# hku-mars/BALM

Measured on AMD Instinct MI355X. Metric: BA iterations/sec (W poses x F plane features), higher is better.
Workload: dtype f64

## Files before the change

balm_amd/csrc/balm_capi.hip:

```cpp
#include <algorithm>
#include <array>
#include <atomic>
#include <chrono>
#include <cmath>
#include <cstdio>
#include <cstdlib>
#include <cstring>

#include "balm_internal.h"

using namespace balm;

#define HIP_TRY(expr)                                                                              \
  do {                                                                                             \
    hipError_t e_ = (expr);                                                                        \
    if (e_ != hipSuccess) {                                                                        \
      ctx->err = std::string(#expr) + ": " + hipGetErrorString(e_);                                \
      return BALM_ERR_HIP;                                                                         \
    }                                                                                              \
  } while (0)

namespace {

#ifdef BALM_COLD_TRACE
// ... 40 lines not shown

static void adopt_warm_ring(balm_ctx *ctx) {
  if (ctx->ring.buf[0] || ctx->device < 0 || ctx->device >= 64) return;
  DeviceWarm &w = g_warm[ctx->device];
  std::lock_guard<std::mutex> lk(w.mu);
  if (!w.started) return;
  if (w.th.joinable()) w.th.join();
  if (w.ring_ready.load(std::memory_order_acquire)) {
    const int key = ctx->ring.pool_key;
    ctx->ring = w.ring; ctx->ring.pool_key = key;
    w.ring = PinnedRing(); w.ring_ready.store(false);
  }
}

struct Span {
  balm_ctx *c; int slot; hipEvent_t a = nullptr, b = nullptr;
  Span(balm_ctx *ctx, int s) : c(ctx), slot(s) {
    if (!c->timer.on) return;
    a = take(); b = take();
    hipEventRecord(a, c->stream);
  }
  ~Span() {
    if (!c->timer.on) return;
    hipEventRecord(b, c->stream);
    c->timer.pending.push_back({a, b, slot});
  }
  hipEvent_t take() {
    if (!c->timer.pool.empty()) { hipEvent_t e = c->timer.pool.back(); c->timer.pool.pop_back(); return e; }
    hipEvent_t e; hipEventCreate(&e); return e;
  }
};

void collect_timing(balm_ctx *c) {
  for (auto &sp : c->timer.pending) {
    float ms = 0;
    if (hipEventElapsedTime(&ms, sp.a, sp.b) == hipSuccess) { c->timer.ms[sp.slot] += ms; c->timer.cnt[sp.slot]++; }
    c->timer.pool.push_back(sp.a); c->timer.pool.push_back(sp.b);
  }
  c->timer.pending.clear();
}

template <class T>
int dalloc(balm_ctx *ctx, T **p, size_t count) {
  if (*p) { hipFree(*p); *p = nullptr; }
  if (count == 0) count = 1;
  HIP_TRY(hipMalloc((void **)p, count * sizeof(T)));
  return BALM_OK;
}

template <class T>
int keep(balm_ctx *ctx, T **p, size_t *cap, size_t count) {
  if (*p && *cap >= count) return BALM_OK;
  for (int k = 0; k < balm_ctx::LM_GRAPHS; k++)
    if (ctx->lm_graph[k]) { hipGraphExecDestroy(ctx->lm_graph[k]); ctx->lm_graph[k] = nullptr; ctx->lm_graph_form[k] = -1; }
// ... 31 lines not shown
  return reinterpret_cast<T *>(ctx->d_stage + off);
}

int sync_stream(balm_ctx *ctx) {
  HIP_TRY(hipStreamSynchronize(ctx->stream));
  HIP_TRY(hipGetLastError());
  collect_timing(ctx);
  return BALM_OK;
}

long red_dacc_off(const balm_ctx *c) { return (long)c->ntiles * TILE_ELEMS; }
long red_r_off(const balm_ctx *c) { return red_dacc_off(c) + (long)DACC_MAX * c->W; }

bool has_transport(const balm_ctx *ctx) { return ctx->comm || multi_is_loopback(ctx) || ctx->allreduce; }

int hook_allreduce(balm_ctx *ctx, double *buf, long n) {
  if (ctx->comm) { Span sp(ctx, BALM_T_COMM); return comm_allreduce(ctx, buf, n); }
  if (multi_is_loopback(ctx)) { Span sp(ctx, BALM_T_COMM); return loopback_allreduce(ctx, buf, n); }
  if (!ctx->allreduce) return BALM_OK;
  int rc = sync_stream(ctx);
  if (rc) return rc;
  if (ctx->allreduce((void *)buf, n, ctx->allreduce_user) != 0) {
    ctx->err = "all-reduce hook failed";
    return BALM_ERR_STATE;
  }
  return BALM_OK;
}

int set_damping(balm_ctx *ctx, double u) {
  ctx->u_value = u;
  ctx->u_on_device = false;
  return BALM_OK;
}
int push_damping(balm_ctx *ctx) {
  double *slot = ctx->h_scal + 16 + (ctx->u_ring++ & 63);
  *slot = ctx->u_value;
  HIP_TRY(hipMemcpyAsync(ctx->d_scal + SCAL_U, slot, sizeof(double), hipMemcpyHostToDevice, ctx->stream));
  ctx->u_on_device = true;
  return BALM_OK;
}

static void collect_timing_if_idle(balm_ctx *ctx) {
  if (!ctx->timer.on || ctx->timer.pending.empty()) return;
  if (hipStreamSynchronize(ctx->stream) == hipSuccess) collect_timing(ctx);
}

int wait_scalars(balm_ctx *ctx) {
  volatile double *stamp = ctx->h_scal + SCAL_STAMP;
  const double want = (double)ctx->mail_seq;
  const auto t0 = std::chrono::steady_clock::now();
  for (int spin = 0;; spin++) {
    if (*stamp == want) { std::atomic_thread_fence(std::memory_order_acquire); collect_timing_if_idle(ctx); return BALM_OK; }
    if ((spin & 255) == 255 && std::chrono::steady_clock::now() - t0 > std::chrono::microseconds(300)) break;
  }
  int rc = sync_stream(ctx);
  if (rc) return rc;
  if (*stamp != want) { ctx->err = "balm_damping_iter: the iteration's scalars did not arrive"; return BALM_ERR_HIP; }
  return BALM_OK;
}

void drop_lm_graphs(balm_ctx *ctx) {
  for (int k = 0; k < balm_ctx::LM_GRAPHS; k++) {
    if (ctx->lm_graph[k]) hipGraphExecDestroy(ctx->lm_graph[k]);
    ctx->lm_graph[k] = nullptr; ctx->lm_graph_form[k] = -1;
  }
}

int residual_device(balm_ctx *ctx, const double *d_poses, int f0, int f1, int slot, bool defer_sum = false, bool send_mail = false) {
  if (f1 <= f0) {
    HIP_TRY(hipMemsetAsync(ctx->d_scal + slot, 0, sizeof(double), ctx->stream));
    ctx->nr_tmp = 0;
  } else {
    Span sp(ctx, BALM_T_MOMENTS);
    launch_world_moments(ctx->stream, ctx->d_cl, d_poses, ctx->W, f0, f1, ctx->d_C);
    const EigenMail mail{ctx->d_scal, ctx->d_hscal, send_mail ? (double)++ctx->mail_seq : 0.0, slot};
    ctx->nr_tmp = launch_feature_eigen(ctx->stream, ctx->d_C, ctx->has_fix ? ctx->d_fix : nullptr, ctx->d_coe, f0, f1, ctx->d_feat_tmp,
                                       ctx->d_rpart_tmp, send_mail ? &mail : nullptr);
    if (!defer_sum) launch_sum_scalar(ctx->stream, ctx->d_rpart_tmp, ctx->nr_tmp, ctx->d_scal + slot);
  }
  HIP_TRY(hipGetLastError());
  if (defer_sum) return BALM_OK;
  return hook_allreduce(ctx, ctx->d_scal + slot, 1);
}

bool fuse_trial(const balm_ctx *ctx) {
  const char *e = getenv("BALM_FUSE_TRIAL");
  return ctx->W <= 256 && ctx->F > 0 && e && e[0] == '1';
}

static bool syrk_int8_mode(const balm_ctx *ctx) {
  if (ctx->flags & BALM_FLAG_SYRK_INT8) return true;
  const char *m = getenv("BALM_SYRK");
  return m && !strcmp(m, "int8");
}
static bool syrk_int8_for(const balm_ctx *ctx, long K) {
  if (!syrk_int8_mode(ctx)) return false;
  if (const char *m = getenv("BALM_SYRK_INT8_MIN_COLS")) return K >= atol(m);
  return K >= 12288L && ctx->W >= 96;
}

int prepare_evaluate(balm_ctx *ctx, int form, int nf) {
  if (nf <= 0) return BALM_OK;
  const SyrkPlan plan = plan_syrk(ctx->ntiles, 3L * nf);
  int rc;
  size_t gcols = (size_t)plan.Kpad + 64, parts = (size_t)plan.SG * ctx->ntiles;
  if (ctx->sparse && nf == ctx->F) {
    gcols = (size_t)ctx->sp_nchunks * ctx->sp_nsteps * 4 + 64;
    parts = (size_t)ctx->sp_nitems;
  }
  {
    const double *before = ctx->d_Gt;
    if ((rc = ensure(ctx, &ctx->d_Gt, &ctx->cap_Gt, gcols * ctx->npad))) return rc;
// ... 6 lines not shown
    if (!ctx->d_rowmax2) ctx->rowmax_trial_valid = false;
    if ((rc = ensure(ctx, &ctx->d_rowmax, &ctx->cap_rowmax, (size_t)ctx->npad + 128))) return rc;
    if ((rc = ensure(ctx, &ctx->d_rowmax2, &ctx->cap_rowmax2, (size_t)ctx->npad + 128))) return rc;
    if ((rc = ensure(ctx, &ctx->d_rowmax_part, &ctx->cap_rowmax_part, (size_t)factors_grid(ctx->W, nf, form) * 6 * ctx->W))) return rc;
    HIP_TRY(prepare_device_syrk_i8());
  }
  if ((rc = ensure(ctx, &ctx->d_dpart, &ctx->cap_dpart, (size_t)factors_grid(ctx->W, nf, form) * DACC_MAX * ctx->W))) return rc;
  if (nf == ctx->F && fuse_trial(ctx)) {
    if (ctx->cap_Gt2 < gcols * ctx->npad || ctx->cap_dpart2 < (size_t)factors_grid(ctx->W, nf, form) * DACC_MAX * ctx->W) ctx->gt_trial_valid = false;
    if ((rc = ensure(ctx, &ctx->d_Gt2, &ctx->cap_Gt2, gcols * ctx->npad))) return rc;
    if ((rc = ensure(ctx, &ctx->d_dpart2, &ctx->cap_dpart2, (size_t)factors_grid(ctx->W, nf, form) * DACC_MAX * ctx->W))) return rc;
  }
  return BALM_OK;
}

int evaluate_device(balm_ctx *ctx, int form, const double *d_poses, int f0, int f1, int slot) {
  const int W = ctx->W, nf = f1 - f0;
  const int dacc = form == 0 ? DACC_LEFT : DACC_RIGHT;
  int rc;
  if (nf <= 0) {
    HIP_TRY(hipMemsetAsync(ctx->d_red, 0, ctx->red_len * sizeof(double), ctx->stream));
    if ((rc = hook_allreduce(ctx, ctx->d_red, (long)ctx->red_len))) return rc;
    Span sp(ctx, BALM_T_ASSEMBLE);
    launch_assemble(ctx->stream, form, ctx->d_red, red_dacc_off(ctx), ctx->d_sub, ctx->ntiles, W, ctx->d_H, ctx->d_g,
                    ctx->d_red + red_r_off(ctx), ctx->d_scal + slot);
    return BALM_OK;
  }
  SyrkPlan plan = plan_syrk(ctx->ntiles, 3L * nf);
  if ((rc = prepare_evaluate(ctx, form, nf))) return rc;
  const int nblk = factors_grid(W, nf, form);
  hipStream_t s = ctx->stream;
  if (!(ctx->feat_cur_valid && f0 == 0 && f1 == ctx->F)) {
    Span sp(ctx, BALM_T_MOMENTS);
    launch_world_moments(s, ctx->d_cl, d_poses, W, f0, f1, ctx->d_C);
    ctx->nr_cur = launch_feature_eigen(s, ctx->d_C, ctx->has_fix ? ctx->d_fix : nullptr, ctx->d_coe, f0, f1, ctx->d_feat, ctx->d_rpart);
    ctx->feat_cur_valid = (f0 == 0 && f1 == ctx->F);
  }
  const int nr = ctx->nr_cur;
  const bool sparse = ctx->sparse && f0 == 0 && f1 == ctx->F;
  const size_t kpad = sparse ? (size_t)ctx->sp_nchunks * ctx->sp_nsteps * 4 : (size_t)plan.Kpad;
  if (!(ctx->gt_cur_valid && ctx->feat_cur_valid && f0 == 0 && f1 == ctx->F)) {
    Span sp(ctx, BALM_T_FACTORS);
    const size_t k0 = (size_t)3 * nf, k1 = kpad + 64;
    if (ctx->gt_dirty_cols == ~(size_t)0) {
      HIP_TRY(hipMemsetAsync(ctx->d_Gt, 0, ctx->cap_Gt * sizeof(double), s));
      ctx->gt_dirty_cols = 0;
    } else if (ctx->gt_dirty_cols > k0) {
      HIP_TRY(hipMemsetAsync(ctx->d_Gt + k0 * ctx->npad, 0, (std::max(ctx->gt_dirty_cols, k1) - k0) * ctx->npad * sizeof(double), s));
    }
    ctx->gt_dirty_cols = k0;
    ctx->rowmax_cur_valid = launch_factors(s, form, ctx->d_cl, d_poses, ctx->d_feat, W, ctx->npad, f0, f1, ctx->d_Gt, ctx->d_dpart, nblk,
                                           sparse ? ctx->d_slot : nullptr, (!sparse && syrk_int8_for(ctx, 3L * nf)) ? ctx->d_rowmax : nullptr, ctx->d_rowmax_part);
    ctx->gt_cur_valid = false;
  }
  HIP_TRY(hipGetLastError());
  const bool int8 = !sparse && syrk_int8_for(ctx, 3L * nf);
  {
    Span sp(ctx, BALM_T_SYRK);
    if (sparse) launch_syrk_sparse(s, ctx->d_Gt, ctx->npad, ctx->d_jobs, ctx->d_items, ctx->d_chunk_ids, ctx->sp_nsteps, ctx->sp_nitems, ctx->d_part);
    else if (int8) {
      if (launch_syrk_i8(s, ctx->d_Gt, ctx->npad, ctx->n, 3L * nf, ctx->d_sub, ctx->ntiles, ctx->d_i8, ctx->d_part,
                         ctx->rowmax_cur_valid ? ctx->d_rowmax : nullptr)) { ctx->err = "INT8 SYRK: unsupported size"; return BALM_ERR_ARG; }
      plan.SG = 1;
    }
    else launch_syrk(s, ctx->d_Gt, ctx->npad, ctx->ntiles, ctx->d_jobs, plan, ctx->d_part);
  }
  {
    Span sp(ctx, BALM_T_ASSEMBLE);
    launch_reduce(s, ctx->d_part, plan.SG, (long)ctx->ntiles * TILE_ELEMS, ctx->d_dpart, nblk, dacc * W,
                  ctx->d_rpart, nr, ctx->d_red, red_dacc_off(ctx), red_r_off(ctx), sparse ? ctx->d_csr : nullptr);
  }
  if ((rc = hook_allreduce(ctx, ctx->d_red, (long)ctx->red_len))) return rc;
  {
    Span sp(ctx, BALM_T_ASSEMBLE);
    launch_assemble(s, form, ctx->d_red, red_dacc_off(ctx), ctx->d_sub, ctx->ntiles, W, ctx->d_H, ctx->d_g, ctx->d_red + red_r_off(ctx),
                    ctx->d_scal + slot);
  }
  return BALM_OK;
}

int trial_device(balm_ctx *ctx, int form, const double *d_poses, int slot) {
  const int W = ctx->W, F = ctx->F;
  hipStream_t s = ctx->stream;
  const SyrkPlan plan = plan_syrk(ctx->ntiles, 3L * F);
  const bool sparse = ctx->sparse;
  const size_t kpad = sparse ? (size_t)ctx->sp_nchunks * ctx->sp_nsteps * 4 : (size_t)plan.Kpad;
  const int nblk = factors_grid(W, F, form);
  {
    Span sp(ctx, BALM_T_FACTORS);
    const size_t k0 = (size_t)3 * F, k1 = kpad + 64;
    HIP_TRY(hipMemsetAsync(ctx->d_Gt2 + k0 * ctx->npad, 0, (k1 - k0) * ctx->npad * sizeof(double), s));
    if (ctx->npad > ctx->n)
      HIP_TRY(hipMemset2DAsync(ctx->d_Gt2 + ctx->n, (size_t)ctx->npad * sizeof(double), 0,
                               (size_t)(ctx->npad - ctx->n) * sizeof(double), k0, s));
    ctx->nr_tmp = launch_moments_factors(s, form, ctx->d_cl, d_poses, ctx->has_fix ? ctx->d_fix : nullptr, ctx->d_coe, W, ctx->npad, F,
                                         ctx->d_Gt2, ctx->d_dpart2, nblk, sparse ? ctx->d_slot : nullptr, ctx->d_feat_tmp, ctx->d_rpart_tmp,
                                         (!sparse && syrk_int8_for(ctx, 3L * F) && ctx->d_rowmax2) ? ctx->d_rowmax2 : nullptr, ctx->d_rowmax_part);
    ctx->rowmax_trial_valid = !sparse && syrk_int8_for(ctx, 3L * F) && ctx->d_rowmax2;
  }
  HIP_TRY(hipGetLastError());
  {
    Span sp(ctx, BALM_T_MOMENTS);
    launch_sum_scalar(s, ctx->d_rpart_tmp, ctx->nr_tmp, ctx->d_scal + slot);
  }
  ctx->gt_trial_valid = true;
  return hook_allreduce(ctx, ctx->d_scal + slot, 1);
}

int read_scalars(balm_ctx *ctx) {
  HIP_TRY(hipMemcpyAsync(ctx->h_scal, ctx->d_scal, 16 * sizeof(double), hipMemcpyDeviceToHost, ctx->stream));
  return sync_stream(ctx);
}

std::vector<unsigned char> obs_of(const double *clusters, int F, int W) {
  std::vector<unsigned char> obs((size_t)F * W);
  parallel_ranges(obs.size(), (size_t)1 << 16, [&](size_t lo, size_t hi) {
    for (size_t t = lo; t < hi; t++) obs[t] = clusters[t * 10 + 9] != 0 ? 1 : 0;
  });
  return obs;
}

// ... 53 lines not shown
  if (hipGetDeviceCount(&ndev) != hipSuccess || ndev < 1 || device < 0 || device >= ndev) return nullptr;
  if (hipSetDevice(device) != hipSuccess) return nullptr;
  cold_mark("balm_create: hipGetDeviceCount + hipSetDevice");
  warm_start(device);
  if (prepare_device_accum() != hipSuccess || prepare_device_cov() != hipSuccess) return nullptr;
  cold_mark("balm_create: prepare_device (function attributes -> code objects)");
  balm_ctx *ctx = new balm_ctx();
  ctx->W = win_size;
  ctx->n = 6 * win_size;
  ctx->npad = (ctx->n + TILE - 1) / TILE * TILE;
  ctx->T = ctx->npad / TILE;
  ctx->nA = (ctx->n + NB - 1) / NB * NB;
  ctx->device = device;
  ctx->flags = flags;
  ctx->timer.on = (flags & BALM_FLAG_TIMING) != 0;
  auto fail = [&]() -> balm_ctx * { one_destroy(ctx); return nullptr; };
  std::vector<int> jobs, sub;
  {
    const int T = ctx->T, ngroups = T / 5;
    std::vector<std::array<int, 3>> mixed[4];
    std::vector<std::array<int, 2>> pairs;
    for (int r = 0; r < TM; r++) for (int c = r; c < TM; c++) pairs.push_back({r, c});
    for (int k = 0; k < 15; k++) mixed[1].push_back({0, pairs[k][0], pairs[k][1]});
    for (int k = 0; k < 10; k++) mixed[1].push_back({1, pairs[k][0], pairs[k][1]});
    for (int k = 10; k < 15; k++) mixed[2].push_back({1, pairs[k][0], pairs[k][1]});
    for (int k = 0; k < 15; k++) mixed[2].push_back({2, pairs[k][0], pairs[k][1]});
    for (int k = 0; k < 5; k++) mixed[2].push_back({3, pairs[k][0], pairs[k][1]});
    for (int k = 5; k < 15; k++) mixed[3].push_back({3, pairs[k][0], pairs[k][1]});
    for (int k = 0; k < 15; k++) mixed[3].push_back({4, pairs[k][0], pairs[k][1]});
    auto regular = [&](int I, int J) {
// ... 54 lines not shown
  if (!ctx) return;
  if (ctx->counted_live) { context_gone(ctx->device); ctx->counted_live = false; }
  comm_destroy(ctx);
  drop_lm_graphs(ctx);
  hipSetDevice(ctx->device);
  if (ctx->stream) hipStreamSynchronize(ctx->stream);
  if (ctx->window) { window_close(ctx->window); ctx->window = nullptr; }
  void *ptrs[] = {ctx->d_cl, ctx->d_fix, ctx->d_coe, ctx->d_poses, ctx->d_poses_tmp, ctx->d_C, ctx->d_feat,
                  ctx->d_Gt, ctx->d_Gt2, ctx->d_dpart2, ctx->d_part, ctx->d_dpart, ctx->d_rpart, ctx->d_feat_tmp, ctx->d_rpart_tmp, ctx->d_red, ctx->d_jobs, ctx->d_sub, ctx->d_H,
                  ctx->d_g, ctx->d_A, ctx->d_Wp, ctx->d_dvec, ctx->d_z, ctx->d_x, ctx->d_perm, ctx->d_dx, ctx->d_scal, ctx->d_arena, ctx->d_pre, ctx->d_flags, ctx->d_minv, ctx->d_macro_tab, ctx->d_trace, ctx->d_slot, ctx->d_items, ctx->d_csr, ctx->d_chunk_ids, ctx->d_stage, ctx->d_i8, ctx->d_rowmax, ctx->d_rowmax2, ctx->d_rowmax_part};
  for (void *p : ptrs) if (p) hipFree(p);
  if (ctx->h_scal) hipHostFree(ctx->h_scal);
  ctx->ring.release();
  if (ctx->amail.host) hipHostFree((void *)ctx->amail.host);
  if (ctx->amail.scan_state) hipFree(ctx->amail.scan_state);
  for (auto &sp : ctx->timer.pending) { hipEventDestroy(sp.a); hipEventDestroy(sp.b); }
  for (auto e : ctx->timer.pool) hipEventDestroy(e);
  if (ctx->stream) hipStreamDestroy(ctx->stream);
  delete ctx;
}

static int build_sparse_plan(balm_ctx *ctx, int F, const unsigned char *obs) {
  ctx->sparse = false;
  const char *mode = getenv("BALM_SYRK");
  if (mode && !strcmp(mode, "dense")) return BALM_OK;
  if (syrk_int8_for(ctx, 3L * F)) return BALM_OK;
  const int W = ctx->W, T = ctx->T, ntiles = ctx->ntiles;
  if (T > 128 || T <= 2 || F < 64) return BALM_OK;
  struct Key { uint64_t hi, lo; int a; };
  std::vector<Key> keys((size_t)F);
  parallel_ranges((size_t)F, (size_t)(65536 / W + 1), [&](size_t a0, size_t a1) {
    for (size_t a = a0; a < a1; a++) {
      uint64_t hi = 0, lo = 0;
      const unsigned char *oa = obs + a * W;
      for (int i = 0; i < W; i++)
        if (oa[i])
          for (int b = (6 * i) / TILE; b <= (6 * i + 5) / TILE; b++) {
            if (b < 64) hi |= 1ull << (63 - b); else lo |= 1ull << (127 - b);
// ... 72 lines not shown
  drop_lm_graphs(ctx);
  ctx->has_fix = fix != nullptr;
  if (fix) {
    if ((rc = keep(ctx, &ctx->d_fix, &ctx->cap_fix, (size_t)F * 10))) return rc;
    HIP_TRY(hipMemcpyAsync(ctx->d_fix, fix, (size_t)F * 10 * sizeof(double), kind, ctx->stream));
  }
  if ((rc = keep(ctx, &ctx->d_coe, &ctx->cap_coe, (size_t)F))) return rc;
  HIP_TRY(hipMemcpyAsync(ctx->d_coe, coeffs, (size_t)F * sizeof(double), kind, ctx->stream));
  if ((rc = keep(ctx, &ctx->d_C, &ctx->cap_C, (size_t)F * 10))) return rc;
  if ((rc = keep(ctx, &ctx->d_feat, &ctx->cap_feat, (size_t)F * FEAT_STRIDE))) return rc;
  if ((rc = keep(ctx, &ctx->d_feat_tmp, &ctx->cap_feat_tmp, (size_t)F * FEAT_STRIDE))) return rc;
  if ((rc = keep(ctx, &ctx->d_rpart, &ctx->cap_rpart, (size_t)(F + 255) / 256 + 1024 + 1))) return rc;
  if ((rc = keep(ctx, &ctx->d_rpart_tmp, &ctx->cap_rpart_tmp, (size_t)(F + 255) / 256 + 1024 + 1))) return rc;
  ctx->feat_cur_valid = false; ctx->gt_cur_valid = false;
  ctx->F = F;
  return BALM_OK;
}

static int assoc_clusters_host(balm_ctx *ctx);

using FillClusters = std::function<void(int, int, double *, unsigned char *)>;

static int one_set_features_fn(balm_ctx *ctx, int F, const FillClusters &fill, const double *fix, const double *coeffs, bool shard_books = false) {
  if (!ctx) return BALM_ERR_ARG;
  if (ctx->multi && F == 0) { ctx->F = 0; ctx->feat_cur_valid = false; ctx->gt_cur_valid = false; ctx->planes_per_pose.clear(); ctx->work_S = ctx->work_B = 0; return BALM_OK; }
  if (F < 1 || !fill || !coeffs) { ctx->err = "balm_set_features: bad argument"; return BALM_ERR_ARG; }
  HIP_TRY(hipSetDevice(ctx->device));
  const int W = ctx->W;
  const size_t count = (size_t)F * W * 10;
  int rc;
// ... 585 lines not shown
  if (!std::isfinite(ctx->h_scal[2]) && !ctx->persistent_off && solve_timed_out(ctx)) {
    ctx->persistent_off = true;
    {
      Span sp(ctx, BALM_T_SOLVE);
      launch_solve(ctx, true);
    }
    HIP_TRY(hipMemcpyAsync(dxi, ctx->d_dx, (size_t)n * sizeof(double), hipMemcpyDeviceToHost, ctx->stream));
    if ((rc = read_scalars(ctx))) return rc;
  }
  if (q1) *q1 = ctx->h_scal[2];
  return BALM_OK;
}

static int lm_enqueue(balm_ctx *ctx, int form, bool evaluated, bool mail) {
  int rc;
  if (evaluated && (rc = evaluate_device(ctx, form, ctx->d_poses, 0, ctx->F, 0))) return rc;
  {
    Span sp(ctx, BALM_T_SOLVE);
    launch_solve(ctx, evaluated, form, ctx->d_poses, ctx->d_poses_tmp);
  }
  ctx->gt_trial_valid = false;
  bool sum_in_mail = false;
  if (fuse_trial(ctx) && ctx->d_Gt2 && ctx->d_dpart2) {
    if ((rc = trial_device(ctx, form, ctx->d_poses_tmp, 1))) return rc;
  } else {
    sum_in_mail = mail && !has_transport(ctx) && ctx->F > 0;
    const bool eigen_mails = sum_in_mail && ctx->F <= 256;
    if ((rc = residual_device(ctx, ctx->d_poses_tmp, 0, ctx->F, 1, sum_in_mail, eigen_mails))) return rc;
    if (eigen_mails) return BALM_OK;
  }
  if (mail) launch_scalars_mail(ctx->stream, ctx->d_scal, ctx->d_hscal, (double)++ctx->mail_seq, sum_in_mail ? ctx->d_rpart_tmp : nullptr,
                                ctx->nr_tmp, 1);
  else HIP_TRY(hipMemcpyAsync(ctx->h_scal, ctx->d_scal, 16 * sizeof(double), hipMemcpyDeviceToHost, ctx->stream));
  return BALM_OK;
}

static int lm_iteration(balm_ctx *ctx, int form, bool evaluated, int it) {
  const char *genv = getenv("BALM_GRAPH");
  const bool disabled = !(genv && (!strcmp(genv, "1") || !strcmp(genv, "debug")));
  const bool graphable = !disabled && ctx->graphs_ok && it >= 1 && !ctx->timer.on && !has_transport(ctx) && !ctx->multi &&
                         ctx->feat_cur_valid && ctx->F > 0 && !solve_is_persistent(ctx);
  if (graphable) {
    const bool fused = fuse_trial(ctx) && ctx->d_Gt2 && ctx->d_dpart2;
    const int slot = (ctx->gt_parity ? 16 : 0) | (fused ? 8 : 0) | (ctx->gt_cur_valid ? 4 : 0) | (evaluated ? 2 : 0) | ctx->parity;
    if (ctx->lm_graph[slot] && ctx->lm_graph_form[slot] != form) {
      hipGraphExecDestroy(ctx->lm_graph[slot]); ctx->lm_graph[slot] = nullptr;
    }
    if (!ctx->lm_graph[slot]) {
      hipGraph_t g = nullptr;
      ctx->u_on_device = true;
      bool ok = hipStreamBeginCapture(ctx->stream, hipStreamCaptureModeThreadLocal) == hipSuccess;
      if (ok) {
        const int rc = lm_enqueue(ctx, form, evaluated, false);
        const hipError_t e = hipStreamEndCapture(ctx->stream, &g);
        ok = rc == BALM_OK && e == hipSuccess && g != nullptr;
      }
      if (ok) ok = hipGraphInstantiate(&ctx->lm_graph[slot], g, nullptr, nullptr, 0) == hipSuccess;
      if (g) hipGraphDestroy(g);
      if (genv && !strcmp(genv, "debug")) fprintf(stderr, "balm_hip: LM graph slot %d capture %s\n", slot, ok ? "ok" : "FAILED");
      if (!ok) {
        hipGetLastError();
        ctx->lm_graph[slot] = nullptr;
        ctx->graphs_ok = false;
      } else {
        ctx->lm_graph_form[slot] = form;
      }
    }
    if (ctx->lm_graph[slot]) {
      int rcu = push_damping(ctx);
      if (rcu) return rcu;
      HIP_TRY(hipGraphLaunch(ctx->lm_graph[slot], ctx->stream));
      return sync_stream(ctx);
    }
    ctx->u_on_device = false;
  }
  int rc = lm_enqueue(ctx, form, evaluated, true);
  if (rc) return rc;
  return wait_scalars(ctx);
}

static int one_damping_iter(balm_ctx *ctx, const balm_lm_opts *o, double *poses, balm_iter_log *log, int *n_iters) {
  if (!ctx) return BALM_ERR_ARG;
  if (!ctx->multi && ctx->F < 1) { ctx->err = "balm_damping_iter: no features installed"; return BALM_ERR_STATE; }
  if (!o || !poses || (o->form != 0 && o->form != 1) || o->max_iter < 1) {
    ctx->err = "balm_damping_iter: bad argument"; return BALM_ERR_ARG;
  }
  if (n_iters) *n_iters = 0;
  HIP_TRY(hipSetDevice(ctx->device));
  const int W = ctx->W, F = ctx->F;
  hipStream_t s = ctx->stream;
  cold_mark("damping_iter: enter");
  int rc = prepare_evaluate(ctx, o->form, F);
// ... 453 lines not shown
  });
}

int balm_get_solve_trace(balm_ctx *ctx, long long *ticks, long capacity, int *dims3) {
  if (!ctx || !dims3) return BALM_ERR_ARG;
  const int P = ctx->nA / NB, RB = 2 * P + 1;
  dims3[0] = RB; dims3[1] = P; dims3[2] = 6;
  if (!ctx->d_trace) { ctx->err = "balm_get_solve_trace: create the context with BALM_SOLVE_TRACE=1 in the environment"; return BALM_ERR_STATE; }
  if (!ticks || capacity < (long)RB * P * 6 + 6L * P) { ctx->err = "balm_get_solve_trace: buffer too small"; return BALM_ERR_ARG; }
  HIP_TRY(hipSetDevice(ctx->device));
  HIP_TRY(hipStreamSynchronize(ctx->stream));
  HIP_TRY(hipMemcpy(ticks, ctx->d_trace, ((size_t)RB * P * 6 + 6 * (size_t)P) * sizeof(long long), hipMemcpyDeviceToHost));
  return BALM_OK;
}

int balm_get_timing(balm_ctx *ctx, double *ms, long *count) {
  if (!ctx) return BALM_ERR_ARG;
  for (int k = 0; k < BALM_T_COUNT; k++) {
    if (ms) ms[k] = ctx->timer.ms[k];
    if (count) count[k] = ctx->timer.cnt[k];
  }
  return BALM_OK;
}

int balm_get_shard_timing(balm_ctx *ctx, int shard, double *ms, long *count) {
  if (!ctx) return BALM_ERR_ARG;
  balm_ctx *q = ctx;
  if (ctx->multi) {
    if (shard < 0 || shard >= ctx->multi->n) { ctx->err = "balm_get_shard_timing: no such shard"; return BALM_ERR_ARG; }
    q = ctx->multi->sub[(size_t)shard];
  } else if (shard != 0) { ctx->err = "balm_get_shard_timing: no such shard"; return BALM_ERR_ARG; }
  return balm_get_timing(q, ms, count);
}

int balm_chain_macro_plan(int panels, int helpers, int *table, long capacity) {
  if (!table || panels < 3 || helpers < 1 || capacity < (long)helpers * 64) return BALM_ERR_ARG;
  std::vector<int> tab;
  if (!balm::chain_macro_plan(panels, helpers, tab)) return BALM_ERR_ARG;
  memcpy(table, tab.data(), tab.size() * sizeof(int));
  return BALM_OK;
}

int balm_reset_timing(balm_ctx *ctx) {
  if (!ctx) return BALM_ERR_ARG;
  for (int k = 0; k < BALM_T_COUNT; k++) { ctx->timer.ms[k] = 0; ctx->timer.cnt[k] = 0; }
  if (balm_multi *m = leader_of(ctx))
    for (size_t q = 1; q < m->sub.size(); q++)
      for (int k = 0; k < BALM_T_COUNT; k++) { m->sub[q]->timer.ms[k] = 0; m->sub[q]->timer.cnt[k] = 0; }
  return BALM_OK;
}

int balm_work_model(balm_ctx *ctx, double *out4) {
  if (!ctx || !out4) return BALM_ERR_ARG;
  const double W = ctx->W, F = ctx->multi ? ctx->multi->F : ctx->F;
  out4[0] = ctx->work_S;
  out4[1] = ctx->work_B;
  if (ctx->multi && ctx->multi->books_per_shard) {
    out4[0] = out4[1] = 0;
    for (const balm_ctx *q : ctx->multi->sub) { out4[0] += q->work_S; out4[1] += q->work_B; }
  }
  (void)W;
  out4[2] = 216.0 * out4[1];
  SyrkPlan p = plan_syrk(ctx->ntiles, 3L * (long)F);
// ... 17 lines not shown
```

balm_amd/csrc/balm_internal.h:

```cpp
#pragma once
#include <hip/hip_runtime.h>
#include <atomic>
#include <condition_variable>
#include <cstddef>
#include <cstdint>
#include <functional>
#include <mutex>
#include <string>
#include <thread>
#include <vector>

#include "../../include/balm_hip.h"
#include "host_stage.h"

namespace balm {

constexpr int TILE = 80;
constexpr int TM = 5;
constexpr int TILE_ELEMS = TILE * TILE;
constexpr int FEAT_STRIDE = 24;
constexpr int DACC_LEFT = 27;
constexpr int DACC_RIGHT = 30;
constexpr int DACC_MAX = 30;
constexpr int NB = 48;
constexpr int MAX_W_LDS = 480;
constexpr int MAX_W = 1024;
constexpr int MAX_SHARDS = 16;

enum { FT_NN = 0, FT_VBAR = 1, FT_LAM = 4, FT_U0 = 7, FT_U1 = 10, FT_U2 = 13, FT_C0 = 16, FT_C1 = 17,
       FT_C2 = 18, FT_COE = 19 };

struct Timer {
  bool on = false;
  struct Span { hipEvent_t a, b; int slot; };
  std::vector<Span> pending;
  std::vector<hipEvent_t> pool;
  double ms[BALM_T_COUNT] = {0};
  long cnt[BALM_T_COUNT] = {0};
};

}

namespace balm {
struct WindowSession;
struct AssocMail {
  volatile unsigned int *host = nullptr; unsigned int *dev = nullptr; unsigned int seq = 0;
  unsigned long long *scan_state = nullptr; unsigned int scan_gen = 0;
};
constexpr long SCAN_TILES_CAP = 8192;
}

struct balm_ctx {
  int W = 0, n = 0, npad = 0, T = 0, ntiles = 0, device = 0, flags = 0;
// ... 49 lines not shown
  double *d_z = nullptr;
  double *d_x = nullptr;
  int *d_perm = nullptr;
  int *d_flags = nullptr;
  long long *d_trace = nullptr;
  int fused_cap = -1;
  int chain_cap = -1;
  double *d_minv = nullptr;
  int *d_macro_tab = nullptr;
  int macro_tab_P = 0, macro_tab_NH = 0;
  double *d_dx = nullptr;
  double *d_scal = nullptr;
  double *h_scal = nullptr;
  double *d_hscal = nullptr;
  unsigned long long mail_seq = 0;
  bool need_minv = false;
  bool solve_tiled = false;
  int chain_refused_P[2] = {-1, -1};
  bool solve_backsub = false;
  bool counted_live = false;
  bool persistent_off = false;
  bool inject_solve_timeout = false;
  bool small_ready = false, small_refused = false;
  double u_value = 0.0;
  bool u_on_device = false;
  int u_ring = 0;
  static constexpr int LM_GRAPHS = 32;
  hipGraphExec_t lm_graph[LM_GRAPHS] = {};
  int lm_graph_form[LM_GRAPHS] = {};
  bool graphs_ok = true;
// ... 32 lines not shown

hipError_t prepare_device_accum();
hipError_t prepare_device_cov();
hipError_t preload_solve();
hipError_t preload_build();
hipError_t preload_voxel();
void launch_transpose_clusters(hipStream_t s, const double *aos, double *soa, int F, int W);
void launch_world_moments(hipStream_t s, const double *cl, const double *poses, int W, int f0, int f1, double *C);
struct EigenMail { double *scal; double *host; double stamp; int slot; };
int launch_feature_eigen(hipStream_t s, const double *C, const double *fix, const double *coe, int f0, int f1,
                         double *feat, double *rpart, const EigenMail *mail = nullptr);
int factors_grid(int W, int nfeat, int form);
int factors_chunk(int W);
bool launch_factors(hipStream_t s, int form, const double *cl, const double *poses, const double *feat, int W,
                    int npad, int f0, int f1, double *Gt, double *dpart, int nblk, const int *slot = nullptr,
                    unsigned long long *rowmax = nullptr, double *rowmax_part = nullptr);
int launch_moments_factors(hipStream_t s, int form, const double *cl, const double *poses, const double *fix, const double *coe, int W,
                           int npad, int F, double *Gt, double *dpart, int nblk, const int *slot, double *feat, double *rpart,
                           unsigned long long *rowmax = nullptr, double *rowmax_part = nullptr);
struct SyrkPlan { int SG; int nsteps; int Kpad; long nblocks; };
SyrkPlan plan_syrk(int ntiles, long K);
void launch_syrk(hipStream_t s, const double *Gt, int npad, int ntiles, const int *tileIJ, const SyrkPlan &p,
                 double *part);
void launch_syrk_sparse(hipStream_t s, const double *Gt, int npad, const int *jobs, const int *items, const int *chunk_ids,
                        int nsteps, long nitems, double *part);
void launch_reduce(hipStream_t s, const double *part, int SG, long tile_elems_total, const double *dpart, int nblk,
                   int dacc_len, const double *rpart, int nr, double *red, long red_dacc_off, long red_r_off,
                   const int *csr_ptr = nullptr);
void launch_assemble(hipStream_t s, int form, const double *red, long red_dacc_off, const int *tileIJ, int ntiles,
                     int W, double *H, double *g, const double *r_in = nullptr, double *r_out = nullptr);
void launch_sum_scalar(hipStream_t s, const double *rpart, int nr, double *out);
// ... 110 lines not shown
```

balm_amd/csrc/kernels_accum.hip:

```cpp
#include "balm_internal.h"

namespace balm {

typedef double d4 __attribute__((ext_vector_type(4)));
typedef double d2 __attribute__((ext_vector_type(2)));

__device__ __forceinline__ double wave_sum(double v) {
#pragma unroll
  for (int off = 32; off > 0; off >>= 1) v += __shfl_xor(v, off, 64);
  return v;
}

struct Obs {
  double N;
  double Rv[3];
  double b[3];
  double Pw[6];
};

__device__ __forceinline__ void to_world(const double P[6], const double v[3], double N, const double R[9],
                                         const double p[3], Obs &o) {
  o.N = N;
#pragma unroll
  for (int r = 0; r < 3; r++) o.Rv[r] = R[r] * v[0] + R[3 + r] * v[1] + R[6 + r] * v[2];
// ... 775 lines not shown
    if (form == 0)
      hipLaunchKernelGGL((k_moments_factors<0, true>), dim3(nblk), dim3(bs), lds, s, cl, poses, fix, coe, W, npad, F, Gt, dpart, slot, feat, rpart, rowmax_part);
    else
      hipLaunchKernelGGL((k_moments_factors<1, true>), dim3(nblk), dim3(bs), lds, s, cl, poses, fix, coe, W, npad, F, Gt, dpart, slot, feat, rpart, rowmax_part);
    hipLaunchKernelGGL(k_rowmax_reduce, dim3((npad + 63) / 64), dim3(1024), 0, s, rowmax_part, nblk, W, npad, rowmax);
    return nblk;
  }
  if (form == 0)
    hipLaunchKernelGGL((k_moments_factors<0, false>), dim3(nblk), dim3(bs), lds, s, cl, poses, fix, coe, W, npad, F, Gt, dpart, slot, feat, rpart, nullptr);
  else
    hipLaunchKernelGGL((k_moments_factors<1, false>), dim3(nblk), dim3(bs), lds, s, cl, poses, fix, coe, W, npad, F, Gt, dpart, slot, feat, rpart, nullptr);
  return nblk;
}

bool launch_factors(hipStream_t s, int form, const double *cl, const double *poses, const double *feat, int W,
                    int npad, int f0, int f1, double *Gt, double *dpart, int nblk, const int *slot, unsigned long long *rowmax, double *rowmax_part) {
  const int Wc = factors_chunk(W), chunks = (W + Wc - 1) / Wc;
  size_t lds = factors_lds(W, form);
  int bs = W <= 64 ? 64 : (W <= 128 ? 128 : 256);
  const int staged = factors_staged(W, f1 - f0, form);
  if (staged) lds += FACTORS_STAGE_BYTES;
  const char *er = getenv("BALM_FACTORS_REGS");
  const bool regs = form == 0 && chunks == 1 && W <= bs && !(er && er[0] == '0');
  if (rowmax && regs) {
    hipLaunchKernelGGL((k_feature_factors<0, true, true>), dim3(nblk, chunks), dim3(bs), lds, s, cl, poses, feat, W, Wc, npad, f0, f1, Gt, dpart, slot, staged, rowmax_part);
    hipLaunchKernelGGL(k_rowmax_reduce, dim3((npad + 63) / 64), dim3(1024), 0, s, rowmax_part, nblk, W, npad, rowmax);
    return true;
  }
#define BALM_FACTORS(F, R) hipLaunchKernelGGL((k_feature_factors<F, R, false>), dim3(nblk, chunks), dim3(bs), lds, s, cl, poses, feat, W, Wc, npad, f0, f1, Gt, dpart, slot, staged, nullptr)
  if (form == 0) { if (regs) BALM_FACTORS(0, true); else BALM_FACTORS(0, false); }
  else BALM_FACTORS(1, false);
#undef BALM_FACTORS
  return false;
}

#include "syrk_mfma_asm.inc"

__device__ __forceinline__ void load5(const double *__restrict__ p, double (&x)[TM]) {
// ... 357 lines not shown
```

include/balm_hip.h:

```cpp
#ifndef BALM_HIP_H
#define BALM_HIP_H

#include <stddef.h>

#ifdef __cplusplus
extern "C" {
#endif

typedef struct balm_ctx balm_ctx;

enum { BALM_FORM_LEFT = 0, BALM_FORM_RIGHT = 1 };

enum {
  BALM_OK = 0,
  BALM_ERR_ARG = 1,
  BALM_ERR_HIP = 2,
  BALM_ERR_STATE = 3,
  BALM_ERR_TOO_FEW_PLANES = 4,
  BALM_ERR_NUMERIC = 5
};

enum {
  BALM_FLAG_TIMING = 1,
  BALM_FLAG_LOOPBACK_SHARDS = 2,
  BALM_FLAG_SYRK_INT8 = 4
};

typedef struct balm_iter_log {
  double r1, r2, u, v, q, q1;
  int accepted;
  int hess_evaluated;
} balm_iter_log;

typedef struct balm_lm_opts {
  int form;
  double u0;
  int max_iter;
  double rel_tol;
  int min_planes_per_pose;
  int force_hess;
  int no_stop;
// ... 119 lines not shown
```

Baseline: 248.2.

## Predictively sleep while waiting for LM scalars, chain timing spans, latch env switches

The host wait for each LM iteration's scalars now uses a per-kind history of iteration durations to sleep until just before the predicted completion, then spins with a pause instruction. The give-up deadline is adapted to that prediction instead of a fixed short window. Timing spans share boundary events and are collected without a full stream sync on every iteration. Environment variables are read once into a switches struct instead of calling getenv on hot paths. The aim is to cut host CPU overhead and sync stalls per iteration, at the risk of oversleeping and adding latency when the prediction is wrong.

```diff
diff --git a/balm_amd/csrc/balm_capi.hip b/balm_amd/csrc/balm_capi.hip
--- a/balm_amd/csrc/balm_capi.hip
+++ b/balm_amd/csrc/balm_capi.hip
@@ -78,16 +78,18 @@
 }
 
 struct Span {
-  balm_ctx *c; int slot; hipEvent_t a = nullptr, b = nullptr;
-  Span(balm_ctx *ctx, int s) : c(ctx), slot(s) {
+  balm_ctx *c; int slot; hipEvent_t *tail; hipEvent_t a = nullptr, b = nullptr; bool owns_a = true;
+  Span(balm_ctx *ctx, int s, hipEvent_t *chain = nullptr) : c(ctx), slot(s), tail(chain) {
     if (!c->timer.on) return;
-    a = take(); b = take();
-    hipEventRecord(a, c->stream);
+    if (tail && *tail) { a = *tail; owns_a = false; }
+    else { a = take(); hipEventRecord(a, c->stream); }
+    b = take();
   }
   ~Span() {
     if (!c->timer.on) return;
     hipEventRecord(b, c->stream);
-    c->timer.pending.push_back({a, b, slot});
+    c->timer.pending.push_back({a, b, slot, owns_a});
+    if (tail) *tail = b;
   }
   hipEvent_t take() {
     if (!c->timer.pool.empty()) { hipEvent_t e = c->timer.pool.back(); c->timer.pool.pop_back(); return e; }
@@ -95,13 +97,26 @@
   }
 };
 
-void collect_timing(balm_ctx *c) {
-  for (auto &sp : c->timer.pending) {
+void collect_timing(balm_ctx *c, size_t count = ~(size_t)0) {
+  auto &pd = c->timer.pending;
+  if (count > pd.size()) count = pd.size();
+  for (size_t k = 0; k < count; k++) {
+    const auto &sp = pd[k];
     float ms = 0;
     if (hipEventElapsedTime(&ms, sp.a, sp.b) == hipSuccess) { c->timer.ms[sp.slot] += ms; c->timer.cnt[sp.slot]++; }
-    c->timer.pool.push_back(sp.a); c->timer.pool.push_back(sp.b);
-  }
-  c->timer.pending.clear();
+    else hipGetLastError();
+    if (sp.owns_a) c->timer.pool.push_back(sp.a);
+    c->timer.pool.push_back(sp.b);
+  }
+  pd.erase(pd.begin(), pd.begin() + (long)count);
+  c->timer.popped += count;
+}
+
+static void collect_timing_before(balm_ctx *c, size_t upto) {
+  if (!c->timer.on || upto <= c->timer.popped) return;
+  const size_t count = upto - c->timer.popped;
+  if (hipEventQuery(c->timer.pending[count - 1].b) == hipSuccess) collect_timing(c, count);
+  else hipGetLastError();
 }
 
 template <class T>
@@ -163,10 +178,11 @@
 
 bool has_transport(const balm_ctx *ctx) { return ctx->comm || multi_is_loopback(ctx) || ctx->allreduce; }
 
-int hook_allreduce(balm_ctx *ctx, double *buf, long n) {
-  if (ctx->comm) { Span sp(ctx, BALM_T_COMM); return comm_allreduce(ctx, buf, n); }
-  if (multi_is_loopback(ctx)) { Span sp(ctx, BALM_T_COMM); return loopback_allreduce(ctx, buf, n); }
+int hook_allreduce(balm_ctx *ctx, double *buf, long n, hipEvent_t *tail = nullptr) {
+  if (ctx->comm) { Span sp(ctx, BALM_T_COMM, tail); return comm_allreduce(ctx, buf, n); }
+  if (multi_is_loopback(ctx)) { Span sp(ctx, BALM_T_COMM, tail); return loopback_allreduce(ctx, buf, n); }
   if (!ctx->allreduce) return BALM_OK;
+  if (tail) *tail = nullptr;
   int rc = sync_stream(ctx);
   if (rc) return rc;
   if (ctx->allreduce((void *)buf, n, ctx->allreduce_user) != 0) {
@@ -189,22 +205,58 @@
   return BALM_OK;
 }
 
-static void collect_timing_if_idle(balm_ctx *ctx) {
-  if (!ctx->timer.on || ctx->timer.pending.empty()) return;
-  if (hipStreamSynchronize(ctx->stream) == hipSuccess) collect_timing(ctx);
+static inline long long mono_ns() {
+  timespec ts;
+  clock_gettime(CLOCK_MONOTONIC, &ts);
+  return (long long)ts.tv_sec * 1000000000LL + ts.tv_nsec;
+}
+
+static inline void cpu_pause() {
+#if defined(__x86_64__) && !defined(__HIP_DEVICE_COMPILE__)
+  __builtin_ia32_pause();
+#else
+  std::atomic_signal_fence(std::memory_order_seq_cst);
+#endif
 }
 
 int wait_scalars(balm_ctx *ctx) {
   volatile double *stamp = ctx->h_scal + SCAL_STAMP;
   const double want = (double)ctx->mail_seq;
-  const auto t0 = std::chrono::steady_clock::now();
+  const int ke = ctx->lm_kind >> 1, kf = ctx->lm_kind & 1;
+  long long &d0 = ctx->lm_last_ns[ke][kf], &d1 = ctx->lm_prev_ns[ke][kf];
+  int &over = ctx->lm_overslept[ke][kf];
+  const bool sample = !ctx->lm_fresh;
+  ctx->lm_fresh = false;
+  const long long t0 = ctx->lm_t0_ns, pred = (d0 > 0 && d1 > 0) ? std::min(d0, d1) : 0;
+  long long give_up = mono_ns() + 300000;
+  bool slept = false;
+  if (pred > 0 && pred < 20000000LL) {
+    give_up = t0 + 4 * pred + 1000000;
+    const long long wake = t0 + pred - 200000;
+    if (wake > mono_ns() + 50000 && *stamp != want) {
+      timespec ts{(time_t)(wake / 1000000000LL), (long)(wake % 1000000000LL)};
+      clock_nanosleep(CLOCK_MONOTONIC, TIMER_ABSTIME, &ts, nullptr);
+      slept = true;
+    }
+  }
   for (int spin = 0;; spin++) {
-    if (*stamp == want) { std::atomic_thread_fence(std::memory_order_acquire); collect_timing_if_idle(ctx); return BALM_OK; }
-    if ((spin & 255) == 255 && std::chrono::steady_clock::now() - t0 > std::chrono::microseconds(300)) break;
+    if (*stamp == want) {
+      std::atomic_thread_fence(std::memory_order_acquire);
+      const long long took = mono_ns() - t0;
+      if (slept && spin == 0) {
+        d0 = d1 = ++over >= 3 ? 0 : std::max(1LL, std::min(pred, took) - 100000);
+        if (d0 == 0) over = 0;
+      } else if (sample) { d1 = d0; d0 = took; over = 0; }
+      if (ctx->timer.pending.size() > Timer::MAX_PENDING && hipStreamSynchronize(ctx->stream) == hipSuccess) collect_timing(ctx);
+      return BALM_OK;
+    }
+    cpu_pause();
+    if ((spin & 63) == 63 && mono_ns() > give_up) break;
   }
   int rc = sync_stream(ctx);
   if (rc) return rc;
   if (*stamp != want) { ctx->err = "balm_damping_iter: the iteration's scalars did not arrive"; return BALM_ERR_HIP; }
+  if (sample) { d1 = d0; d0 = mono_ns() - t0; over = 0; }
   return BALM_OK;
 }
 
@@ -215,12 +267,14 @@
   }
 }
 
-int residual_device(balm_ctx *ctx, const double *d_poses, int f0, int f1, int slot, bool defer_sum = false, bool send_mail = false) {
+int residual_device(balm_ctx *ctx, const double *d_poses, int f0, int f1, int slot, bool defer_sum = false, bool send_mail = false,
+                    hipEvent_t *tail = nullptr) {
   if (f1 <= f0) {
+    if (tail) *tail = nullptr;
     HIP_TRY(hipMemsetAsync(ctx->d_scal + slot, 0, sizeof(double), ctx->stream));
     ctx->nr_tmp = 0;
   } else {
-    Span sp(ctx, BALM_T_MOMENTS);
+    Span sp(ctx, BALM_T_MOMENTS, tail);
     launch_world_moments(ctx->stream, ctx->d_cl, d_poses, ctx->W, f0, f1, ctx->d_C);
     const EigenMail mail{ctx->d_scal, ctx->d_hscal, send_mail ? (double)++ctx->mail_seq : 0.0, slot};
     ctx->nr_tmp = launch_feature_eigen(ctx->stream, ctx->d_C, ctx->has_fix ? ctx->d_fix : nullptr, ctx->d_coe, f0, f1, ctx->d_feat_tmp,
@@ -229,22 +283,30 @@
   }
   HIP_TRY(hipGetLastError());
   if (defer_sum) return BALM_OK;
-  return hook_allreduce(ctx, ctx->d_scal + slot, 1);
-}
-
-bool fuse_trial(const balm_ctx *ctx) {
-  const char *e = getenv("BALM_FUSE_TRIAL");
-  return ctx->W <= 256 && ctx->F > 0 && e && e[0] == '1';
-}
-
-static bool syrk_int8_mode(const balm_ctx *ctx) {
-  if (ctx->flags & BALM_FLAG_SYRK_INT8) return true;
-  const char *m = getenv("BALM_SYRK");
-  return m && !strcmp(m, "int8");
+  return hook_allreduce(ctx, ctx->d_scal + slot, 1, tail);
+}
+
+bool fuse_trial(const balm_ctx *ctx) { return ctx->W <= 256 && ctx->F > 0 && ctx->sw.fuse_trial; }
+
+void latch_switches(balm_ctx *ctx) {
+  Switches sw;
+  const char *e = getenv("BALM_GRAPH");
+  sw.graph_debug = e && !strcmp(e, "debug");
+  sw.graph = sw.graph_debug || (e && !strcmp(e, "1"));
+  e = getenv("BALM_FUSE_TRIAL");
+  sw.fuse_trial = e && e[0] == '1';
+  e = getenv("BALM_FACTORS_REGS");
+  sw.factors_regs = !(e && e[0] == '0');
+  e = getenv("BALM_SYRK");
+  sw.syrk_int8 = (ctx->flags & BALM_FLAG_SYRK_INT8) || (e && !strcmp(e, "int8"));
+  e = getenv("BALM_SYRK_INT8_MIN_COLS");
+  sw.int8_min_set = e != nullptr;
+  sw.int8_min_cols = e ? atol(e) : 0;
+  ctx->sw = sw;
 }
 static bool syrk_int8_for(const balm_ctx *ctx, long K) {
-  if (!syrk_int8_mode(ctx)) return false;
-  if (const char *m = getenv("BALM_SYRK_INT8_MIN_COLS")) return K >= atol(m);
+  if (!ctx->sw.syrk_int8) return false;
+  if (ctx->sw.int8_min_set) return K >= ctx->sw.int8_min_cols;
   return K >= 12288L && ctx->W >= 96;
 }
 
@@ -281,14 +343,17 @@
   return BALM_OK;
 }
 
-int evaluate_device(balm_ctx *ctx, int form, const double *d_poses, int f0, int f1, int slot) {
+int evaluate_device(balm_ctx *ctx, int form, const double *d_poses, int f0, int f1, int slot, hipEvent_t *tail = nullptr) {
+  hipEvent_t own_tail = nullptr;
+  if (!tail) tail = &own_tail;
   const int W = ctx->W, nf = f1 - f0;
   const int dacc = form == 0 ? DACC_LEFT : DACC_RIGHT;
   int rc;
   if (nf <= 0) {
+    *tail = nullptr;
     HIP_TRY(hipMemsetAsync(ctx->d_red, 0, ctx->red_len * sizeof(double), ctx->stream));
-    if ((rc = hook_allreduce(ctx, ctx->d_red, (long)ctx->red_len))) return rc;
-    Span sp(ctx, BALM_T_ASSEMBLE);
+    if ((rc = hook_allreduce(ctx, ctx->d_red, (long)ctx->red_len, tail))) return rc;
+    Span sp(ctx, BALM_T_ASSEMBLE, tail);
     launch_assemble(ctx->stream, form, ctx->d_red, red_dacc_off(ctx), ctx->d_sub, ctx->ntiles, W, ctx->d_H, ctx->d_g,
                     ctx->d_red + red_r_off(ctx), ctx->d_scal + slot);
     return BALM_OK;
@@ -298,7 +363,7 @@
   const int nblk = factors_grid(W, nf, form);
   hipStream_t s = ctx->stream;
   if (!(ctx->feat_cur_valid && f0 == 0 && f1 == ctx->F)) {
-    Span sp(ctx, BALM_T_MOMENTS);
+    Span sp(ctx, BALM_T_MOMENTS, tail);
     launch_world_moments(s, ctx->d_cl, d_poses, W, f0, f1, ctx->d_C);
     ctx->nr_cur = launch_feature_eigen(s, ctx->d_C, ctx->has_fix ? ctx->d_fix : nullptr, ctx->d_coe, f0, f1, ctx->d_feat, ctx->d_rpart);
     ctx->feat_cur_valid = (f0 == 0 && f1 == ctx->F);
@@ -307,7 +372,7 @@
   const bool sparse = ctx->sparse && f0 == 0 && f1 == ctx->F;
   const size_t kpad = sparse ? (size_t)ctx->sp_nchunks * ctx->sp_nsteps * 4 : (size_t)plan.Kpad;
   if (!(ctx->gt_cur_valid && ctx->feat_cur_valid && f0 == 0 && f1 == ctx->F)) {
-    Span sp(ctx, BALM_T_FACTORS);
+    Span sp(ctx, BALM_T_FACTORS, tail);
     const size_t k0 = (size_t)3 * nf, k1 = kpad + 64;
     if (ctx->gt_dirty_cols == ~(size_t)0) {
       HIP_TRY(hipMemsetAsync(ctx->d_Gt, 0, ctx->cap_Gt * sizeof(double), s));
@@ -317,13 +382,14 @@
     }
     ctx->gt_dirty_cols = k0;
     ctx->rowmax_cur_valid = launch_factors(s, form, ctx->d_cl, d_poses, ctx->d_feat, W, ctx->npad, f0, f1, ctx->d_Gt, ctx->d_dpart, nblk,
-                                           sparse ? ctx->d_slot : nullptr, (!sparse && syrk_int8_for(ctx, 3L * nf)) ? ctx->d_rowmax : nullptr, ctx->d_rowmax_part);
+                                           sparse ? ctx->d_slot : nullptr, (!sparse && syrk_int8_for(ctx, 3L * nf)) ? ctx->d_rowmax : nullptr, ctx->d_rowmax_part,
+                                           ctx->sw.factors_regs);
     ctx->gt_cur_valid = false;
   }
   HIP_TRY(hipGetLastError());
   const bool int8 = !sparse && syrk_int8_for(ctx, 3L * nf);
   {
-    Span sp(ctx, BALM_T_SYRK);
+    Span sp(ctx, BALM_T_SYRK, tail);
     if (sparse) launch_syrk_sparse(s, ctx->d_Gt, ctx->npad, ctx->d_jobs, ctx->d_items, ctx->d_chunk_ids, ctx->sp_nsteps, ctx->sp_nitems, ctx->d_part);
     else if (int8) {
       if (launch_syrk_i8(s, ctx->d_Gt, ctx->npad, ctx->n, 3L * nf, ctx->d_sub, ctx->ntiles, ctx->d_i8, ctx->d_part,
@@ -333,20 +399,20 @@
     else launch_syrk(s, ctx->d_Gt, ctx->npad, ctx->ntiles, ctx->d_jobs, plan, ctx->d_part);
   }
   {
-    Span sp(ctx, BALM_T_ASSEMBLE);
+    Span sp(ctx, BALM_T_ASSEMBLE, tail);
     launch_reduce(s, ctx->d_part, plan.SG, (long)ctx->ntiles * TILE_ELEMS, ctx->d_dpart, nblk, dacc * W,
                   ctx->d_rpart, nr, ctx->d_red, red_dacc_off(ctx), red_r_off(ctx), sparse ? ctx->d_csr : nullptr);
   }
-  if ((rc = hook_allreduce(ctx, ctx->d_red, (long)ctx->red_len))) return rc;
+  if ((rc = hook_allreduce(ctx, ctx->d_red, (long)ctx->red_len, tail))) return rc;
   {
-    Span sp(ctx, BALM_T_ASSEMBLE);
+    Span sp(ctx, BALM_T_ASSEMBLE, tail);
     launch_assemble(s, form, ctx->d_red, red_dacc_off(ctx), ctx->d_sub, ctx->ntiles, W, ctx->d_H, ctx->d_g, ctx->d_red + red_r_off(ctx),
                     ctx->d_scal + slot);
   }
   return BALM_OK;
 }
 
-int trial_device(balm_ctx *ctx, int form, const double *d_poses, int slot) {
+int trial_device(balm_ctx *ctx, int form, const double *d_poses, int slot, hipEvent_t *tail = nullptr) {
   const int W = ctx->W, F = ctx->F;
   hipStream_t s = ctx->stream;
   const SyrkPlan plan = plan_syrk(ctx->ntiles, 3L * F);
@@ -354,7 +420,7 @@
   const size_t kpad = sparse ? (size_t)ctx->sp_nchunks * ctx->sp_nsteps * 4 : (size_t)plan.Kpad;
   const int nblk = factors_grid(W, F, form);
   {
-    Span sp(ctx, BALM_T_FACTORS);
+    Span sp(ctx, BALM_T_FACTORS, tail);
     const size_t k0 = (size_t)3 * F, k1 = kpad + 64;
     HIP_TRY(hipMemsetAsync(ctx->d_Gt2 + k0 * ctx->npad, 0, (k1 - k0) * ctx->npad * sizeof(double), s));
     if (ctx->npad > ctx->n)
@@ -367,11 +433,11 @@
   }
   HIP_TRY(hipGetLastError());
   {
-    Span sp(ctx, BALM_T_MOMENTS);
+    Span sp(ctx, BALM_T_MOMENTS, tail);
     launch_sum_scalar(s, ctx->d_rpart_tmp, ctx->nr_tmp, ctx->d_scal + slot);
   }
   ctx->gt_trial_valid = true;
-  return hook_allreduce(ctx, ctx->d_scal + slot, 1);
+  return hook_allreduce(ctx, ctx->d_scal + slot, 1, tail);
 }
 
 int read_scalars(balm_ctx *ctx) {
@@ -455,6 +521,7 @@
   ctx->device = device;
   ctx->flags = flags;
   ctx->timer.on = (flags & BALM_FLAG_TIMING) != 0;
+  latch_switches(ctx);
   auto fail = [&]() -> balm_ctx * { one_destroy(ctx); return nullptr; };
   std::vector<int> jobs, sub;
   {
@@ -539,7 +606,7 @@
   ctx->ring.release();
   if (ctx->amail.host) hipHostFree((void *)ctx->amail.host);
   if (ctx->amail.scan_state) hipFree(ctx->amail.scan_state);
-  for (auto &sp : ctx->timer.pending) { hipEventDestroy(sp.a); hipEventDestroy(sp.b); }
+  for (auto &sp : ctx->timer.pending) { if (sp.owns_a) hipEventDestroy(sp.a); hipEventDestroy(sp.b); }
   for (auto e : ctx->timer.pool) hipEventDestroy(e);
   if (ctx->stream) hipStreamDestroy(ctx->stream);
   delete ctx;
@@ -547,6 +614,7 @@
 
 static int build_sparse_plan(balm_ctx *ctx, int F, const unsigned char *obs) {
   ctx->sparse = false;
+  latch_switches(ctx);
   const char *mode = getenv("BALM_SYRK");
   if (mode && !strcmp(mode, "dense")) return BALM_OK;
   if (syrk_int8_for(ctx, 3L * F)) return BALM_OK;
@@ -649,6 +717,8 @@
   if ((rc = keep(ctx, &ctx->d_rpart_tmp, &ctx->cap_rpart_tmp, (size_t)(F + 255) / 256 + 1024 + 1))) return rc;
   ctx->feat_cur_valid = false; ctx->gt_cur_valid = false;
   ctx->F = F;
+  for (int k = 0; k < 4; k++) { ctx->lm_last_ns[k >> 1][k & 1] = ctx->lm_prev_ns[k >> 1][k & 1] = 0; ctx->lm_overslept[k >> 1][k & 1] = 0; }
+  ctx->lm_fresh = true;
   return BALM_OK;
 }
 
@@ -1264,19 +1334,20 @@
 
 static int lm_enqueue(balm_ctx *ctx, int form, bool evaluated, bool mail) {
   int rc;
-  if (evaluated && (rc = evaluate_device(ctx, form, ctx->d_poses, 0, ctx->F, 0))) return rc;
+  hipEvent_t tail = nullptr;
+  if (evaluated && (rc = evaluate_device(ctx, form, ctx->d_poses, 0, ctx->F, 0, &tail))) return rc;
   {
-    Span sp(ctx, BALM_T_SOLVE);
+    Span sp(ctx, BALM_T_SOLVE, &tail);
     launch_solve(ctx, evaluated, form, ctx->d_poses, ctx->d_poses_tmp);
   }
   ctx->gt_trial_valid = false;
   bool sum_in_mail = false;
   if (fuse_trial(ctx) && ctx->d_Gt2 && ctx->d_dpart2) {
-    if ((rc = trial_device(ctx, form, ctx->d_poses_tmp, 1))) return rc;
+    if ((rc = trial_device(ctx, form, ctx->d_poses_tmp, 1, &tail))) return rc;
   } else {
     sum_in_mail = mail && !has_transport(ctx) && ctx->F > 0;
     const bool eigen_mails = sum_in_mail && ctx->F <= 256;
-    if ((rc = residual_device(ctx, ctx->d_poses_tmp, 0, ctx->F, 1, sum_in_mail, eigen_mails))) return rc;
+    if ((rc = residual_device(ctx, ctx->d_poses_tmp, 0, ctx->F, 1, sum_in_mail, eigen_mails, &tail))) return rc;
     if (eigen_mails) return BALM_OK;
   }
   if (mail) launch_scalars_mail(ctx->stream, ctx->d_scal, ctx->d_hscal, (double)++ctx->mail_seq, sum_in_mail ? ctx->d_rpart_tmp : nullptr,
@@ -1286,8 +1357,7 @@
 }
 
 static int lm_iteration(balm_ctx *ctx, int form, bool evaluated, int it) {
-  const char *genv = getenv("BALM_GRAPH");
-  const bool disabled = !(genv && (!strcmp(genv, "1") || !strcmp(genv, "debug")));
+  const bool disabled = !ctx->sw.graph;
   const bool graphable = !disabled && ctx->graphs_ok && it >= 1 && !ctx->timer.on && !has_transport(ctx) && !ctx->multi &&
                          ctx->feat_cur_valid && ctx->F > 0 && !solve_is_persistent(ctx);
   if (graphable) {
@@ -1307,7 +1377,7 @@
       }
       if (ok) ok = hipGraphInstantiate(&ctx->lm_graph[slot], g, nullptr, nullptr, 0) == hipSuccess;
       if (g) hipGraphDestroy(g);
-      if (genv && !strcmp(genv, "debug")) fprintf(stderr, "balm_hip: LM graph slot %d capture %s\n", slot, ok ? "ok" : "FAILED");
+      if (ctx->sw.graph_debug) fprintf(stderr, "balm_hip: LM graph slot %d capture %s\n", slot, ok ? "ok" : "FAILED");
       if (!ok) {
         hipGetLastError();
         ctx->lm_graph[slot] = nullptr;
@@ -1324,8 +1394,12 @@
     }
     ctx->u_on_device = false;
   }
+  ctx->lm_t0_ns = mono_ns();
+  ctx->lm_kind = (evaluated ? 2 : 0) | (ctx->feat_cur_valid ? 1 : 0);
+  const size_t spans_before = ctx->timer.popped + ctx->timer.pending.size();
   int rc = lm_enqueue(ctx, form, evaluated, true);
   if (rc) return rc;
+  collect_timing_before(ctx, spans_before);
   return wait_scalars(ctx);
 }
 
@@ -1809,8 +1883,15 @@
   return BALM_OK;
 }
 
+static void drain_timing(balm_ctx *ctx) {
+  if (ctx->timer.pending.empty()) return;
+  if (hipSetDevice(ctx->device) == hipSuccess && hipStreamSynchronize(ctx->stream) == hipSuccess) collect_timing(ctx);
+  else hipGetLastError();
+}
+
 int balm_get_timing(balm_ctx *ctx, double *ms, long *count) {
   if (!ctx) return BALM_ERR_ARG;
+  drain_timing(ctx);
   for (int k = 0; k < BALM_T_COUNT; k++) {
     if (ms) ms[k] = ctx->timer.ms[k];
     if (count) count[k] = ctx->timer.cnt[k];
@@ -1838,10 +1919,13 @@
 
 int balm_reset_timing(balm_ctx *ctx) {
   if (!ctx) return BALM_ERR_ARG;
+  drain_timing(ctx);
   for (int k = 0; k < BALM_T_COUNT; k++) { ctx->timer.ms[k] = 0; ctx->timer.cnt[k] = 0; }
   if (balm_multi *m = leader_of(ctx))
-    for (size_t q = 1; q < m->sub.size(); q++)
+    for (size_t q = 1; q < m->sub.size(); q++) {
+      drain_timing(m->sub[q]);
       for (int k = 0; k < BALM_T_COUNT; k++) { m->sub[q]->timer.ms[k] = 0; m->sub[q]->timer.cnt[k] = 0; }
+    }
   return BALM_OK;
 }
 
diff --git a/balm_amd/csrc/balm_internal.h b/balm_amd/csrc/balm_internal.h
--- a/balm_amd/csrc/balm_internal.h
+++ b/balm_amd/csrc/balm_internal.h
@@ -32,11 +32,22 @@
 
 struct Timer {
   bool on = false;
-  struct Span { hipEvent_t a, b; int slot; };
+  struct Span { hipEvent_t a, b; int slot; bool owns_a; };
   std::vector<Span> pending;
+  size_t popped = 0;
   std::vector<hipEvent_t> pool;
   double ms[BALM_T_COUNT] = {0};
   long cnt[BALM_T_COUNT] = {0};
+  static constexpr size_t MAX_PENDING = 512;
+};
+
+struct Switches {
+  bool graph = false, graph_debug = false;
+  bool fuse_trial = false;
+  bool factors_regs = true;
+  bool syrk_int8 = false;
+  bool int8_min_set = false;
+  long int8_min_cols = 0;
 };
 
 }
@@ -116,6 +127,11 @@
   double *h_scal = nullptr;
   double *d_hscal = nullptr;
   unsigned long long mail_seq = 0;
+  long long lm_t0_ns = 0, lm_last_ns[2][2] = {{0, 0}, {0, 0}}, lm_prev_ns[2][2] = {{0, 0}, {0, 0}};
+  int lm_overslept[2][2] = {{0, 0}, {0, 0}};
+  bool lm_fresh = true;
+  int lm_kind = 0;
+  balm::Switches sw;
   bool need_minv = false;
   bool solve_tiled = false;
   int chain_refused_P[2] = {-1, -1};
@@ -178,7 +194,8 @@
 int factors_chunk(int W);
 bool launch_factors(hipStream_t s, int form, const double *cl, const double *poses, const double *feat, int W,
                     int npad, int f0, int f1, double *Gt, double *dpart, int nblk, const int *slot = nullptr,
-                    unsigned long long *rowmax = nullptr, double *rowmax_part = nullptr);
+                    unsigned long long *rowmax = nullptr, double *rowmax_part = nullptr,
+                    bool allow_regs = true);
 int launch_moments_factors(hipStream_t s, int form, const double *cl, const double *poses, const double *fix, const double *coe, int W,
                            int npad, int F, double *Gt, double *dpart, int nblk, const int *slot, double *feat, double *rpart,
                            unsigned long long *rowmax = nullptr, double *rowmax_part = nullptr);
diff --git a/balm_amd/csrc/kernels_accum.hip b/balm_amd/csrc/kernels_accum.hip
--- a/balm_amd/csrc/kernels_accum.hip
+++ b/balm_amd/csrc/kernels_accum.hip
@@ -813,14 +813,14 @@
 }
 
 bool launch_factors(hipStream_t s, int form, const double *cl, const double *poses, const double *feat, int W,
-                    int npad, int f0, int f1, double *Gt, double *dpart, int nblk, const int *slot, unsigned long long *rowmax, double *rowmax_part) {
+                    int npad, int f0, int f1, double *Gt, double *dpart, int nblk, const int *slot, unsigned long long *rowmax, double *rowmax_part,
+                    bool allow_regs) {
   const int Wc = factors_chunk(W), chunks = (W + Wc - 1) / Wc;
   size_t lds = factors_lds(W, form);
   int bs = W <= 64 ? 64 : (W <= 128 ? 128 : 256);
   const int staged = factors_staged(W, f1 - f0, form);
   if (staged) lds += FACTORS_STAGE_BYTES;
-  const char *er = getenv("BALM_FACTORS_REGS");
-  const bool regs = form == 0 && chunks == 1 && W <= bs && !(er && er[0] == '0');
+  const bool regs = form == 0 && chunks == 1 && W <= bs && allow_regs;
   if (rowmax && regs) {
     hipLaunchKernelGGL((k_feature_factors<0, true, true>), dim3(nblk, chunks), dim3(bs), lds, s, cl, poses, feat, W, Wc, npad, f0, f1, Gt, dpart, slot, staged, rowmax_part);
     hipLaunchKernelGGL(k_rowmax_reduce, dim3((npad + 63) / 64), dim3(1024), 0, s, rowmax_part, nblk, W, npad, rowmax);
diff --git a/include/balm_hip.h b/include/balm_hip.h
--- a/include/balm_hip.h
+++ b/include/balm_hip.h
@@ -25,6 +25,7 @@
   BALM_FLAG_LOOPBACK_SHARDS = 2,
   BALM_FLAG_SYRK_INT8 = 4
 };
+
 
 typedef struct balm_iter_log {
   double r1, r2, u, v, q, q1;
```

Measured after the change: 249.6 (median of 6 runs). About the same (+0.6%).
